# andvg3/LipVQ-VAE

Hardware: AMD Instinct MI355X
Metric: actions tokenized/sec (encode+quantize) at B=4096 T=128 K=1024, 1/2/4/8 GPU (higher is better)
Workload: dtype f32

## Files before the change

### lipvq-vae_amd/csrc/lipvq_screen.h

```cpp
#ifndef LIPVQ_SCREEN_H_
#define LIPVQ_SCREEN_H_
#include <hip/hip_fp16.h>

#include <type_traits>

#include "lipvq_common.h"

typedef _Float16 f16x8 __attribute__((ext_vector_type(8)));

#define LIPVQ_SCREEN_GAMMA 3.814697265625e-06f
#define SCREEN_WAVES 8

struct PrepLayout {
    int S, Dpad, Kpad, ntiles;
    size_t o_hdr, o_mu, o_tiles, tile_bytes, total;
    size_t o_tiles_hi, tile_bytes_hi;
};

#define LIPVQ_SCREEN_GAMMA_WIDE 1.52587890625e-05f
#define LQ_SCREEN_NARROW_MAX_S 13

__host__ __device__ static inline int lq_screen_S(int D) {
    const int s = (D + 15) / 16;
    return D <= 0 ? 0 : s <= 2 ? 2 : s <= 4 ? 4 : s <= 8 ? 8 : s <= 13 ? 13 : s <= 16 ? 16 : s <= 24 ? 24 : s <= 32 ? 32 : 0;
}
__host__ __device__ static inline float lq_screen_gamma(int D) {
    return lq_screen_S(D) > LQ_SCREEN_NARROW_MAX_S ? LIPVQ_SCREEN_GAMMA_WIDE : LIPVQ_SCREEN_GAMMA;
}

__host__ __device__ static inline PrepLayout prep_layout(int K, int D) {
    PrepLayout L;
    L.S = lq_screen_S(D) ? lq_screen_S(D) : (D + 15) / 16;
    L.Dpad = L.S * 16;
    L.Kpad = ((K + 31) / 32) * 32;
    L.ntiles = ((L.Kpad / 32 + 7) / 8) * 8;
    L.o_hdr = 0;
    L.o_mu = 64;
    L.o_tiles = L.o_mu + sizeof(float) * (size_t)L.Dpad;
    L.o_tiles = (L.o_tiles + 255) & ~(size_t)255;
    L.tile_bytes = (size_t)L.S * 2048 + 256;
    L.o_tiles_hi = (L.o_tiles + (size_t)L.ntiles * L.tile_bytes + 255) & ~(size_t)255;
    L.tile_bytes_hi = (size_t)L.S * 1024 + 256;
    L.total = L.o_tiles_hi + (size_t)L.ntiles * L.tile_bytes_hi;
    return L;
}


__device__ __forceinline__ int lq_scale_exp(float maxabs) {
    const int e = (int)((__float_as_uint(maxabs) >> 23) & 0xff) - 127;
    int k = 13 - e;
    k = k < -60 ? -60 : k;
    k = k > 60 ? 60 : k;
    return (maxabs > 0.0f && maxabs < INFINITY) ? k : 0;
}
__device__ __forceinline__ float lq_pow2f(int k) { return __uint_as_float((unsigned)(k + 127) << 23); }

constexpr int screen_default_tc(int S) { return (S <= 2) ? 8 : (S <= 4) ? 4 : (S <= 8) ? 2 : 1; }

template <int S, int TC_ = screen_default_tc(S), bool COARSE = false>
struct ScreenCfg {
    static constexpr int FRAG_BYTES = COARSE ? S * 1024 : S * 2048;
    static constexpr int TILE_BYTES = FRAG_BYTES + 256;
    static constexpr int TC = TC_;
    static constexpr int STAGE_BYTES = TC * TILE_BYTES;
    static constexpr int STAGE_VEC = STAGE_BYTES / 16;
};

template <int S>
struct StandaloneScreen {
    static constexpr int TC = (S <= 2) ? 4 : (S <= 4) ? 2 : 1;
    static constexpr int NB = (S <= 8) ? 4 : 3;
    static constexpr bool PACK = S <= 4;
};

template <bool PACK>
__device__ __forceinline__ void lq_track_one(float v, int id, unsigned keep_mask, float& m1, float& m2, int& k1) {
    if constexpr (PACK) {
        float key;
        asm("v_and_or_b32 %0, %1, %2, %3" : "=v"(key) : "v"(v), "s"(keep_mask), "v"(id));
        m2 = __builtin_amdgcn_fmed3f(key, m1, m2);
        asm("v_min_f32 %0, %1, %2" : "=v"(m1) : "v"(key), "v"(m1));
    } else {
        const bool lt = v < m1;
        k1 = lt ? id : k1;
        m2 = __builtin_amdgcn_fmed3f(v, m1, m2);
        m1 = lt ? v : m1;
    }
}

__device__ __forceinline__ float lq_coarse_zn(float a2lo, float n2, float fz, float fown, float rho) {
    const float A = lq_sqrt(a2lo), B = lq_sqrt(n2) * fz;
    const float t = lq_fma(rho, lq_fma(3.0f, A, B), A);
    return t * (fown / fz) * 1.0009765625f;
}
template <int LO, int HI, bool PACK = false, bool COARSE = false>
__device__ __forceinline__ void lq_track_part(const f32x16& acc, float e2, float en, const float (&frow)[16], const float (&znr)[16],
                                              int id, unsigned keep_mask, float (&m1)[16], float (&m2)[16], int (&k1)[16]) {
#pragma unroll
    for (int r = LO; r < HI; ++r) {
        const float v = COARSE ? acc[r] : lq_fma(e2, frow[r], acc[r]);
        lq_track_one<PACK>(v, id, keep_mask, m1[r], m2[r], k1[r]);
    }
}

template <int S, bool PACK, bool COARSE = false>
__device__ __forceinline__ void lq_track_after_mfma(int j, const f32x16& acc, float e2, float en, const float (&frow)[16],
                                                    const float (&znr)[16], int id, unsigned keep_mask, float (&m1)[16],
                                                    float (&m2)[16], int (&k1)[16]) {
    constexpr int NM = COARSE ? S : 3 * S;
    const int lo = (16 * j) / NM, hi = (16 * (j + 1)) / NM;
#pragma unroll
    for (int r = 0; r < 16; ++r)
        if (r >= lo && r < hi) {
            const float v = COARSE ? acc[r] : lq_fma(e2, frow[r], acc[r]);
            lq_track_one<PACK>(v, id, keep_mask, m1[r], m2[r], k1[r]);
        }
}

template <int N>
__device__ __forceinline__ void lq_wait_vmcnt() {
    static_assert(N >= 0 && N < 64, "vmcnt immediate");
    asm volatile("s_waitcnt vmcnt(%0)" ::"n"(N) : "memory");
}
template <int S, int TC_, int NB>
constexpr size_t lq_ring_bytes() { return (size_t)NB * ScreenCfg<S, TC_>::STAGE_BYTES + 1024; }

__host__ __device__ static inline int lq_pack_bits(int ntiles) { int b = 1; while ((1 << b) < ntiles) ++b; return b; }

struct LqNoDeferred { __device__ __forceinline__ void operator()() const {} };
template <int BASE, int NDEF, int NPF>
__device__ __forceinline__ void lq_wait_vmcnt_deferred(bool cd, bool cp) {
    static_assert(BASE + NDEF + NPF < 64, "vmcnt immediate");
    if (NDEF > 0 && NPF > 0 && cd && cp) lq_wait_vmcnt<BASE + NDEF + NPF>();
    else if (NDEF > 0 && cd) lq_wait_vmcnt<BASE + NDEF>();
    else if (NPF > 0 && cp) lq_wait_vmcnt<BASE + NPF>();
    else lq_wait_vmcnt<BASE>();
}
template <int S, int NT, int TC_ = screen_default_tc(S), int NB = 4, bool PACK = false, bool COARSE = false, int NDEF = 0,
          typename DEFERRED = LqNoDeferred, int NPF = 0>
__device__ __forceinline__ void lq_screen_core(const f16x8 (&ah)[S], const f16x8 (&al)[S],
                                               const unsigned char* __restrict__ tiles, int ntiles,
                                               unsigned char* stage0, int tid, const float (&frow)[16], const float (&znr)[16],
                                               float (&m1)[16], float (&m2)[16], int (&k1)[16],
                                               bool have_def = false, DEFERRED deferred = DEFERRED(), bool wave_def = true,
                                               bool have_pf = false) {
    using C = ScreenCfg<S, TC_, COARSE>;
    static_assert(NB >= 3 && NB <= 4, "ring of 3 or 4 stage buffers");
    constexpr int NW = NT / 64;
    constexpr int CHUNKS = (C::STAGE_BYTES + 1023) / 1024;
    constexpr int CPW = (CHUNKS + NW - 1) / NW;
    constexpr int PD = NB - 1;
    constexpr int NSTEP = C::TC * S;
    constexpr int MID = (C::TC >= 2) ? (C::TC / 2) * S : S / 2;
    constexpr int FR = 2;
    constexpr int FD = FR - 1;
    constexpr int PERIOD = ((C::TC & 1) || (NSTEP % FR)) ? 2 : 1;
    static_assert(C::STAGE_BYTES >= 1024 && C::STAGE_BYTES % 16 == 0, "stage copies are whole KiB pieces");
    static_assert(NSTEP - FD >= MID, "next-stage fragments are read after the hand-over");
    static_assert(CPW * PD < 64, "vmcnt immediate");
    const int lane = tid & 63, ln = lane & 31;
    const int wave = __builtin_amdgcn_readfirstlane(tid >> 6);
    const int nstage = ntiles / C::TC;
    unsigned char* dummy = stage0 + (size_t)NB * C::STAGE_BYTES;
    typedef __attribute__((address_space(3))) void* lds_ptr_t;
    typedef const __attribute__((address_space(1))) void* glb_ptr_t;
    auto stage_dma = [&](int st, int buf) {
        const bool real = st < nstage;
        const unsigned char* src = tiles + (real ? (size_t)st * C::STAGE_BYTES : (size_t)0);
        unsigned char* dst = stage0 + (size_t)buf * C::STAGE_BYTES;
#pragma unroll
        for (int j = 0; j < CPW; ++j) {
            int chunk = wave + j * NW;
            chunk = chunk < CHUNKS ? chunk : CHUNKS - 1;
            int off = chunk * 1024;
            off = off + 1024 <= C::STAGE_BYTES ? off : C::STAGE_BYTES - 1024;
            unsigned char* d = real ? dst + off : dummy;
            __builtin_amdgcn_global_load_lds((glb_ptr_t)(src + off + lane * 16), (lds_ptr_t)d, 16, 0, 0);
        }
    };
    auto frag = [&](const unsigned char* tb, int s, int hl) {
        return COARSE ? *reinterpret_cast<const f16x8*>(tb + ((size_t)s * 64 + lane) * 16)
                      : *reinterpret_cast<const f16x8*>(tb + (((size_t)s * 2 + hl) * 64 + lane) * 16);
    };
    lq_wg_barrier();
#pragma unroll
    for (int p = 0; p < PD; ++p) stage_dma(p, p);
    static_assert((PD - 1) * CPW + NDEF + NPF < 64, "vmcnt immediate");
    const bool count_def = NDEF > 0 && have_def && wave_def;
    const bool count_pf = NPF > 0 && have_pf;
    if ((NDEF > 0 && have_def) || count_pf) deferred();
    lq_wait_vmcnt_deferred<(PD - 1) * CPW, NDEF, NPF>(count_def, count_pf);
    lq_wg_barrier();

    f32x16 accA, accB;
#pragma unroll
    for (int r = 0; r < 16; ++r) accB[r] = INFINITY;
    float e2A = 0.0f, e2B = 0.0f;
    int codeA = 0, codeB = 0;
    const unsigned keep_mask = PACK ? ~((1u << lq_pack_bits(ntiles)) - 1u) : 0xffffffffu;
    f16x8 fh[FR], fl[FR];
    float e2q[2] = {0.0f, 0.0f};
    float enq[2] = {0.0f, 0.0f};
    float enA = 0.0f, enB = 0.0f;
#pragma unroll
    for (int g = 0; g < FD; ++g) {
        fh[g] = frag(stage0, g, 0);
        if constexpr (!COARSE) fl[g] = frag(stage0, g, 1);
    }
    e2q[0] = reinterpret_cast<const float*>(stage0 + C::FRAG_BYTES)[ln];
    if constexpr (COARSE) enq[0] = reinterpret_cast<const float*>(stage0 + C::FRAG_BYTES + 128)[ln];
    static_assert(FD <= S, "prologue reads stay in tile 0");
    int buf = 0;
    auto do_stage = [&](auto POS, int st) {
        constexpr int par = (decltype(POS)::value * C::TC) & 1;
        constexpr int so = (decltype(POS)::value * NSTEP) % FR;
        const unsigned char* sb = stage0 + (size_t)buf * C::STAGE_BYTES;
        int nbuf = buf + 1; nbuf = nbuf == NB ? 0 : nbuf;
        const unsigned char* nsb = stage0 + (size_t)nbuf * C::STAGE_BYTES;
#pragma unroll
        for (int g = 0; g < NSTEP; ++g) {
            const int c = g / S, s = g % S;
            if (g == MID) {
                if ((count_def || count_pf) && st == 0) lq_wait_vmcnt_deferred<(PD >= 2 ? (PD - 2) * CPW : 0), (PD >= 2 ? NDEF : 0), (PD >= 2 ? NPF : 0)>(count_def, count_pf);
                else lq_wait_vmcnt<(PD >= 2 ? (PD - 2) * CPW : 0)>();
                lq_wg_barrier();
                int b = buf + PD; b = b >= NB ? b - NB : b;
                stage_dma(st + PD, b);
            }
            f32x16& acc = (((c + par) & 1) == 0) ? accA : accB;
            const f32x16& prev = (((c + par) & 1) == 0) ? accB : accA;
            const float e2_prev = (((c + par) & 1) == 0) ? e2B : e2A;
            const float en_prev = (((c + par) & 1) == 0) ? enB : enA;
            const int code_prev = (((c + par) & 1) == 0) ? codeB : codeA;
            if (s == 0) {
                const float e2c = e2q[(c + par) & 1];
                const float enc = enq[(c + par) & 1];
#pragma unroll
                for (int r = 0; r < 16; ++r) acc[r] = COARSE ? lq_fma(-znr[r], enc, e2c * frow[r]) : 0.0f;
                int code = PACK ? (st * C::TC + c) : (st * C::TC + c) * 32 + ln;
                if constexpr (PACK) asm volatile("" : "+v"(code));
                if (((c + par) & 1) == 0) { e2A = e2c; enA = enc; codeA = code; } else { e2B = e2c; enB = enc; codeB = code; }
            }
            const f16x8 bh = fh[(g + so) % FR];
            f16x8 bl = bh;
            if constexpr (!COARSE) bl = fl[(g + so) % FR];
            auto read_ahead = [&]() {
                const int g1 = g + FD;
                const unsigned char* base = (g1 < NSTEP) ? sb : nsb;
                const int gg = (g1 < NSTEP) ? g1 : g1 - NSTEP;
                const unsigned char* tb = base + (size_t)(gg / S) * C::TILE_BYTES;
                fh[(g1 + so) % FR] = frag(tb, gg % S, 0);
                if constexpr (!COARSE) fl[(g1 + so) % FR] = frag(tb, gg % S, 1);
                if (gg % S == 0) {
                    e2q[(g1 / S + par) & 1] = reinterpret_cast<const float*>(tb + C::FRAG_BYTES)[ln];
                    if constexpr (COARSE) enq[(g1 / S + par) & 1] = reinterpret_cast<const float*>(tb + C::FRAG_BYTES + 128)[ln];
                }
            };
            __builtin_amdgcn_sched_barrier(0);
            acc = __builtin_amdgcn_mfma_f32_32x32x16_f16(ah[s], bh, acc, 0, 0, 0);
            __builtin_amdgcn_sched_barrier(0);
            read_ahead();
            __builtin_amdgcn_sched_barrier(0);
            lq_track_after_mfma<S, PACK, COARSE>(COARSE ? s : 3 * s + 0, prev, e2_prev, en_prev, frow, znr, code_prev, keep_mask, m1, m2, k1);
            __builtin_amdgcn_sched_barrier(0);
            if constexpr (!COARSE) {
                acc = __builtin_amdgcn_mfma_f32_32x32x16_f16(al[s], bh, acc, 0, 0, 0);
                lq_track_after_mfma<S, PACK>(3 * s + 1, prev, e2_prev, en_prev, frow, znr, code_prev, keep_mask, m1, m2, k1);
                __builtin_amdgcn_sched_barrier(0);
                acc = __builtin_amdgcn_mfma_f32_32x32x16_f16(ah[s], bl, acc, 0, 0, 0);
                lq_track_after_mfma<S, PACK>(3 * s + 2, prev, e2_prev, en_prev, frow, znr, code_prev, keep_mask, m1, m2, k1);
                __builtin_amdgcn_sched_barrier(0);
            }
        }
        buf = nbuf;
    };
    for (int st = 0; st < nstage; st += PERIOD) {
        do_stage(std::integral_constant<int, 0>{}, st);
        if constexpr (PERIOD == 2) do_stage(std::integral_constant<int, 1>{}, st + 1);
    }
    lq_track_part<0, 16, PACK, COARSE>(accB, e2B, enB, frow, znr, codeB, keep_mask, m1, m2, k1);
    lq_wait_vmcnt<0>();
    lq_wg_barrier();
}


__device__ __forceinline__ void lq_row_factors(float fown, int lane, float (&frow)[16]) {
    const int h = lane >> 5;
#pragma unroll
    for (int r = 0; r < 16; ++r) frow[r] = __shfl(fown, (r & 3) + 8 * (r >> 2) + 4 * h, 64);
}

#define LQ_DECIDE_STRIDE 36
#define LQ_DECIDE_BYTES (32 * LQ_DECIDE_STRIDE * 4)

struct LqDecision {
    float vv[16];
    float m2min, best, t0, p;
    bool screen_ok;
};

template <bool PACK = false, bool COARSE = false>
__device__ __forceinline__ bool lq_screen_decide(const float (&m1)[16], const float (&m2)[16], const int (&k1)[16],
                                                 unsigned char* wave_lds ,
                                                 const unsigned* hdr, float n2, float fown, float gamma, int K, int D,
                                                 int lane, int& my_k, LqDecision& dec, float pack_eps = 0.0f,
                                                 unsigned keep_mask = 0xffffffffu, float zn = 0.0f,
                                                 const unsigned char* tiles = nullptr, size_t tile_bytes = 0, int frag_bytes = 0) {
    constexpr int TS = LQ_DECIDE_STRIDE;
    const int ln = lane & 31, h = lane >> 5;
    float* tv = reinterpret_cast<float*>(wave_lds);
#pragma unroll
    for (int r = 0; r < 16; ++r) tv[((r & 3) + 8 * (r >> 2) + 4 * h) * TS + ln] = m1[r];
    __builtin_amdgcn_s_waitcnt(0xC07F);
    __builtin_amdgcn_wave_barrier();
    float best = INFINITY, second = INFINITY;
    int pos = 0;
    {
        const float4* pv = reinterpret_cast<const float4*>(tv + ln * TS + 16 * h);
#pragma unroll
        for (int q = 0; q < 4; ++q) {
            const float4 v4 = pv[q];
            const float vv[4] = {v4.x, v4.y, v4.z, v4.w};
#pragma unroll
            for (int e = 0; e < 4; ++e) {
                dec.vv[4 * q + e] = vv[e];
                const bool take = vv[e] < best;
                second = __builtin_amdgcn_fmed3f(vv[e], best, second);
                pos = take ? 4 * q + e : pos;
                best = take ? vv[e] : best;
            }
        }
    }
    __builtin_amdgcn_wave_barrier();
#pragma unroll
    for (int r = 0; r < 16; ++r) tv[((r & 3) + 8 * (r >> 2) + 4 * h) * TS + ln] = m2[r];
    __builtin_amdgcn_s_waitcnt(0xC07F);
    __builtin_amdgcn_wave_barrier();
    float m2min = INFINITY;
    {
        const float4* pv = reinterpret_cast<const float4*>(tv + ln * TS + 16 * h);
#pragma unroll
        for (int q = 0; q < 4; ++q) {
            const float4 v4 = pv[q];
            m2min = fminf(m2min, fminf(fminf(v4.x, v4.y), fminf(v4.z, v4.w)));
        }
    }
    second = fminf(second, m2min);
    __builtin_amdgcn_wave_barrier();
    int bk;
    if constexpr (PACK) {
        bk = (int)(__float_as_uint(best) & ~keep_mask) * 32 + 16 * h + pos;
    } else {
        int* tk = reinterpret_cast<int*>(wave_lds);
#pragma unroll
        for (int r = 0; r < 16; ++r) tk[((r & 3) + 8 * (r >> 2) + 4 * h) * TS + ln] = k1[r];
        __builtin_amdgcn_s_waitcnt(0xC07F);
        __builtin_amdgcn_wave_barrier();
        bk = tk[ln * TS + 16 * h + pos];
    }
    {
        const float ob = __shfl_xor(best, 32, 64);
        const float os = __shfl_xor(second, 32, 64);
        const int ok = __shfl_xor(bk, 32, 64);
        second = fminf(fminf(second, os), fmaxf(best, ob));
        const bool take = ob < best;
        bk = take ? ok : bk;
        best = take ? ob : best;
    }
    __builtin_amdgcn_wave_barrier();
    my_k = bk;
    const float E2max = __uint_as_float(hdr[0]);
    const float Emax = lq_sqrt(__uint_as_float(hdr[1]));
    const float twoemax = __uint_as_float(hdr[2]);
    const float cross = 2.0f * lq_sqrt(n2) * Emax;
    const int Dpad16 = ((D + 15) / 16) * 16 + ((D & 7) ? 88 : 0);
    const float u24 = 5.9604644775390625e-08f;
    const float eps_s = gamma * (E2max + cross) * fown;
    const float n2s = n2 * fown;
    float w2 = 0.0f;
    if constexpr (COARSE) {
        const int bkc = (bk >= 0 && bk < K) ? bk : 0;
        const float en = reinterpret_cast<const float*>(tiles + (size_t)(bkc >> 5) * tile_bytes + (size_t)frag_bytes + 128)[bkc & 31];
        w2 = 2.0f * zn * en;
        w2 = lq_fma(w2, 9.5367431640625e-07f, w2);
    }
    const float s1 = fmaxf(0.0f, best + w2 + n2s) + eps_s + (float)(Dpad16 + 2) * u24 * n2s;
    dec.t0 = w2 + 2.0f * eps_s + 2.125f * (float)(Dpad16 / 8 + 12) * u24 * s1;
    dec.p = 2.125f * pack_eps;
    dec.best = best;
    dec.m2min = m2min;
    dec.screen_ok = (twoemax < INFINITY) && (bk >= 0) && (bk < K);
    const float thr = dec.t0 + dec.p * (lq_abs(best) + lq_abs(second));
    return dec.screen_ok && (second - best > thr);
}

#define LQ_CAND_MAX 6

#define LQ_STREAM2_MIN_S 9
struct LqWorkspace {
    unsigned char* base;
    int64_t N;
    int D;

    static constexpr int kHeaderBytes = 64, kLive = 8, kSlot2 = kLive + 2;
    __host__ __device__ static inline LqWorkspace from_lists(int* row_list, int64_t N) {
        return LqWorkspace{reinterpret_cast<unsigned char*>(row_list) - kHeaderBytes, N, 0};
    }
    __host__ __device__ static inline LqWorkspace from_live(int* live) {
        return LqWorkspace{reinterpret_cast<unsigned char*>(live - kLive), 0, 0};
    }
    __host__ __device__ static inline size_t list_ints(int64_t N) { return ((size_t)N + 15) & ~(size_t)15; }
    __host__ __device__ static inline size_t short_cap(int64_t N) { return (size_t)N + 64; }
    __host__ __device__ static inline size_t w2q_floats(int D) {
        return (D + 15) / 16 >= LQ_STREAM2_MIN_S ? (size_t)((D + 31) / 32) * 16 * 256 : 0;
    }
    __host__ __device__ static inline size_t lists_end(int64_t N) {
        return kHeaderBytes + sizeof(int) * (3 * list_ints(N) + 16 * short_cap(N));
    }
    __host__ __device__ static inline size_t nearest_bytes(int64_t N) { return lists_end(N); }
    __host__ __device__ static inline size_t tokenize_bytes(int64_t N, int D) {
        return lists_end(N) + sizeof(float) * w2q_floats(D) + 256 + sizeof(float) * (size_t)N * (size_t)D;
    }

    __host__ __device__ inline int* header() const { return reinterpret_cast<int*>(base); }
    __host__ __device__ inline int* published() const { return header(); }
    __host__ __device__ inline const int* listed() const { return header() + 1; }
    __host__ __device__ inline int* live() const { return header() + kLive; }
    __host__ __device__ inline int* slot2_count() const { return header() + kSlot2; }
    __host__ __device__ inline int* row_list() const { return reinterpret_cast<int*>(base + kHeaderBytes); }
    __host__ __device__ inline int* best_list() const { return row_list() + list_ints(N); }
    __host__ __device__ inline int* short_lists() const { return row_list() + 2 * list_ints(N); }
    __host__ __device__ inline size_t short_cap() const { return short_cap(N); }
    __host__ __device__ inline int* slot2_list() const { return row_list() + (2 * list_ints(N) + 16 * short_cap(N)); }
    __host__ __device__ inline float* w2q() const { return reinterpret_cast<float*>(base + lists_end(N)); }
    __host__ __device__ inline float* ze_scratch() const {
        return reinterpret_cast<float*>(base + ((lists_end(N) + sizeof(float) * w2q_floats(D) + 255) & ~(size_t)255));
    }
    __host__ __device__ inline long long* stamps() const { return reinterpret_cast<long long*>(row_list() + (N / 2 & ~1)); }
};

#if defined(__HIPCC__)
__device__ __forceinline__ void lq_ws_begin(int* __restrict__ live) {
    if (blockIdx.x == 0 && threadIdx.x == 0) *LqWorkspace::from_live(live).slot2_count() = 0;
}
__device__ __forceinline__ void lq_ws_publish(int* __restrict__ live) {
    asm volatile("s_waitcnt vmcnt(0)" ::: "memory");
    __syncthreads();
    if (threadIdx.x == 0) {
        const unsigned long long old = atomicAdd(reinterpret_cast<unsigned long long*>(live), 1ull << 32);
        if ((unsigned)(old >> 32) == gridDim.x - 1u) {
            const int listed = (int)(unsigned)old;
            int* published = LqWorkspace::from_live(live).published();
            published[0] = listed;
            published[1] = listed;
            *reinterpret_cast<unsigned long long*>(live) = 0ull;
        }
    }
}
__device__ __forceinline__ int lq_ws_reserve(int* __restrict__ live, int n) {
    return (int)(unsigned)atomicAdd(reinterpret_cast<unsigned long long*>(live), (unsigned long long)(unsigned)n);
}
#endif

template <bool PACK>
__device__ __forceinline__ void lq_emit_candidates(const LqDecision& dec, bool lists_ok, int K, int lane, unsigned keep_mask,
                                                   const unsigned char* wave_lds, int& head, unsigned& mask_out,
                                                   int (&codes)[LQ_CAND_MAX]) {
    const int ln = lane & 31, h = lane >> 5;
    const float ab = lq_abs(dec.best);
    const float vmax0 = (dec.best + dec.t0 + dec.p * ab) / (1.0f - dec.p);
    const float vmax = vmax0 + lq_abs(vmax0) * 9.5367431640625e-07f + 1.1754944e-38f;
    int n = 0;
    unsigned mask = 0u;
    bool nothing = !lists_ok || !dec.screen_ok || !(vmax == vmax);
    const bool second_in = !(dec.m2min - dec.best > dec.t0 + dec.p * (ab + lq_abs(dec.m2min)));
#pragma unroll
    for (int q = 0; q < LQ_CAND_MAX; ++q) codes[q] = 0;
#pragma unroll
    for (int e = 0; e < 16; ++e) {
        const float v = dec.vv[e];
        if (!(v > vmax)) mask |= 1u << e;
        if (!(v - dec.best > dec.t0 + dec.p * (ab + lq_abs(v)))) {
            int code;
            if constexpr (PACK) code = (int)(__float_as_uint(v) & ~keep_mask) * 32 + 16 * h + e;
            else code = reinterpret_cast<const int*>(wave_lds)[ln * LQ_DECIDE_STRIDE + 16 * h + e];
            nothing = nothing || code < 0 || code >= K;
#pragma unroll
            for (int q = 0; q < LQ_CAND_MAX; ++q)
                if (q == n) codes[q] = code;
            ++n;
        }
    }
    head = nothing ? -1 : ((second_in || n > LQ_CAND_MAX) ? -2 : n);
    mask_out = mask;
}

__device__ __forceinline__ void lq_emit_store(bool need, int slot , int head, unsigned mask,
                                              const int (&codes)[LQ_CAND_MAX], int my_k, int64_t row, int* __restrict__ amb_list,
                                              int64_t N, int lane) {
    const int h = lane >> 5;
    const LqWorkspace ws = LqWorkspace::from_lists(amb_list, N);
    if (h == 0 && need) {
        ws.row_list()[slot] = (int)row;
        ws.best_list()[slot] = my_k;
    }
    if (!need || (size_t)slot >= ws.short_cap()) return;
    int* out = ws.short_lists() + (size_t)slot * 16 + 8 * h;
    static_assert(LQ_CAND_MAX == 6, "a part is {n, mask, six codes}");
    typedef int lq_i4 __attribute__((ext_vector_type(4)));
    lq_i4* out4 = reinterpret_cast<lq_i4*>(out);
    out4[0] = lq_i4{head, (int)mask, codes[0], codes[1]};
    out4[1] = lq_i4{codes[2], codes[3], codes[4], codes[5]};
}

#define LQ_SLOT_HEAD(cl, h) ((cl)[8 * (h)])
#define LQ_SLOT_SHORT(n0, n1) ((n0) >= 0 && (n1) >= 0 && (n0) + (n1) >= 1 && (n0) <= LQ_CAND_MAX && (n1) <= LQ_CAND_MAX)
#define LQ_SLOT_CODE(cl, n0, j) ((j) < (n0) ? (cl)[2 + (j)] : (cl)[10 + ((j) - (n0))])
#define LQ_SLOT_FIRST(cl, n0) ((cl)[(n0) > 0 ? 2 : 10])
#define LQ_SLOT_LANES(cl) (((unsigned)(cl)[1] & 0xffffu) | (((unsigned)(cl)[9] & 0xffffu) << 16))

template <bool PACK>
__device__ __forceinline__ void lq_screen_emit(const LqDecision& dec, bool certified, bool lists_ok, int my_k, int64_t row,
                                               bool row_valid, int* __restrict__ amb_count, int* __restrict__ amb_list, int64_t N,
                                               int K, int lane, unsigned keep_mask, const unsigned char* wave_lds) {
    const bool need = row_valid && !certified;
    if (__builtin_amdgcn_ballot_w64(need) == 0ull) return;
    const int ln = lane & 31, h = lane >> 5;
    const unsigned long long lm = __builtin_amdgcn_ballot_w64(h == 0 && need);
    const int leader = __builtin_ctzll(lm);
    int base = 0;
    if (lane == leader) base = lq_ws_reserve(amb_count, __builtin_popcountll(lm));
    int head;
    unsigned mask;
    int codes[LQ_CAND_MAX];
    lq_emit_candidates<PACK>(dec, lists_ok, K, lane, keep_mask, wave_lds, head, mask, codes);
    base = __shfl(base, leader, 64);
    int slot = base + __builtin_popcountll(lm & ((1ull << lane) - 1ull));
    slot = __shfl(slot, ln, 64);
    lq_emit_store(need, slot, head, mask, codes, my_k, row, amb_list, N, lane);
}

#define LQ_LISTS_ALL_K 2048
template <int DCH, int DIST, typename ZLOAD>
__device__ __forceinline__ int lq_lists_row(ZLOAD zload, const float* __restrict__ cb, int K, const int* cl, int lane, bool all_here) {
    constexpr int D = DCH * 8;
    const int g = lane >> 3, j = lane & 7;
    int n0 = -1, n1 = -1;
    if (cl) { n0 = LQ_SLOT_HEAD(cl, 0); n1 = LQ_SLOT_HEAD(cl, 1); }
    const bool shortlist = LQ_SLOT_SHORT(n0, n1);
    const bool lanescan = !shortlist && n0 != -1 && n1 != -1 && (n0 == -2 || n1 == -2 || n0 > LQ_CAND_MAX || n1 > LQ_CAND_MAX);
    const unsigned lmask = lanescan ? LQ_SLOT_LANES(cl) : 0u;
    bool scan_here = lanescan && lmask != 0u && __builtin_popcount(lmask) * ((K + 31) / 32) <= 128;
    unsigned lm_eff = lmask;
    if (!shortlist && !scan_here) {
        if (!all_here) return -1;
        scan_here = true;
        lm_eff = (lanescan && lmask != 0u) ? lmask : 0xffffffffu;
    }
    const bool scanning = !shortlist;
    const int P = scanning ? __builtin_popcount(lm_eff) : 0;
    const int nc = scanning ? P * ((K + 31) / 32) : n0 + n1;
    float zv[DCH];
#pragma unroll
    for (int i = 0; i < DCH; ++i) zv[i] = zload(8 * i + j);
    float best_v = INFINITY;
    int best_k = 0x7fffffff;
    for (int c0 = 0; c0 < nc; c0 += 8) {
        const int ci = c0 + g;
        bool live = ci < nc;
        int code;
        if (scanning) {
            const int t = ci / P, w = ci - t * P;
            unsigned m = lm_eff;
            for (int q = 0; q < w; ++q) m &= m - 1;
            code = 32 * t + __builtin_ctz(m | 0x80000000u);
            live = live && code < K;
        } else {
            code = live ? LQ_SLOT_CODE(cl, n0, ci) : LQ_SLOT_FIRST(cl, n0);
        }
        code = (code >= 0 && code < K) ? code : 0;
        const float* c = cb + (size_t)code * D;
        float s;
        if constexpr (DIST == LIPVQ_DIST_NORM) {
            float a = 0.0f;
#pragma unroll
            for (int i = 0; i < DCH; ++i) { const float d = zv[i] - c[8 * i + j]; a = lq_fma(d, d, a); }
            s = __shfl(a, 8 * g, 64);
#pragma unroll
            for (int l = 1; l < 8; ++l) s = s + __shfl(a, 8 * g + l, 64);
            s = lq_sqrt(s);
        } else {
            float acc[4] = {0.f, 0.f, 0.f, 0.f};
#pragma unroll
            for (int i = 0; i < DCH; ++i) {
                const int q = (i < (DCH / 4) * 4) ? (i & 3) : 0;
                const float d = zv[i] - c[8 * i + j];
                acc[q] = acc[q] + d * d;
            }
            const float vl = ((acc[0] + acc[1]) + acc[2]) + acc[3];
            s = __shfl(vl, 8 * g, 64);
#pragma unroll
            for (int l = 1; l < 8; ++l) s = s + __shfl(vl, 8 * g + l, 64);
        }
        const float v = (live && s == s) ? s : INFINITY;
        const int kk = live ? code : 0x7fffffff;
        LQ_TAKE_MIN(best_v, best_k, v, kk);
    }
    LQ_WAVE_MIN(best_v, best_k, 8);
    if (best_k < 0 || best_k >= K) {
        const int fb = scanning ? __builtin_ctz(lm_eff) : LQ_SLOT_FIRST(cl, n0);
        best_k = (fb >= 0 && fb < K) ? fb : 0;
    }
    return best_k;
}

template <bool PACK, int DCH, int DIST, int NKEEP = 0>
__device__ __forceinline__ bool lq_screen_decide_inplace(const LqDecision& dec, bool certified, bool lists_ok, int& my_k, int64_t row0,
                                                         bool row_valid, int* __restrict__ amb_count, const float* __restrict__ z,
                                                         const float* __restrict__ cb, int K, int lane, unsigned keep_mask,
                                                         unsigned char* wave_lds ,
                                                         const f32x16* zkeep = nullptr) {
    const bool need = row_valid && !certified;
    if (__builtin_amdgcn_ballot_w64(need) == 0ull) return certified;
    const int ln = lane & 31, h = lane >> 5;
    unsigned long long lm = __builtin_amdgcn_ballot_w64(h == 0 && need);
    if (lane == __builtin_ctzll(lm)) (void)lq_ws_reserve(amb_count, __builtin_popcountll(lm));
    int head;
    unsigned mask;
    int codes[LQ_CAND_MAX];
    lq_emit_candidates<PACK>(dec, lists_ok, K, lane, keep_mask, wave_lds, head, mask, codes);
    __builtin_amdgcn_wave_barrier();
    int* parts = reinterpret_cast<int*>(wave_lds);
    static_assert(LQ_CAND_MAX == 6 && 32 * 16 * 4 <= LQ_DECIDE_BYTES, "a part is {n, mask, six codes}");
    if (need) {
        typedef int lq_i4 __attribute__((ext_vector_type(4)));
        lq_i4* out4 = reinterpret_cast<lq_i4*>(parts + ln * 16 + 8 * h);
        out4[0] = lq_i4{head, (int)mask, codes[0], codes[1]};
        out4[1] = lq_i4{codes[2], codes[3], codes[4], codes[5]};
    }
    __builtin_amdgcn_s_waitcnt(0xC07F);
    __builtin_amdgcn_wave_barrier();
    constexpr int D = DCH * 8;
    while (lm) {
        const int r = __builtin_ctzll(lm);
        lm &= lm - 1ull;
        int bk;
        if constexpr (NKEEP > 0) {
            static_assert(NKEEP * 32 == D, "the kept tiles are the row");
            float* zrow = reinterpret_cast<float*>(wave_lds + LQ_DECIDE_BYTES);
            if (ln == r) {
#pragma unroll
                for (int t = 0; t < NKEEP; ++t)
#pragma unroll
                    for (int q = 0; q < 16; ++q) zrow[32 * t + 2 * q + h] = zkeep[t][q];
            }
            __builtin_amdgcn_s_waitcnt(0xC07F);
            __builtin_amdgcn_wave_barrier();
            bk = lq_lists_row<DCH, DIST>([&](int f) { return zrow[f]; }, cb, K, parts + r * 16, lane, true);
            __builtin_amdgcn_wave_barrier();
        } else {
            const float* zr = z + (size_t)(row0 + r) * D;
            bk = lq_lists_row<DCH, DIST>([&](int f) { return __hip_atomic_load(zr + f, __ATOMIC_RELAXED, __HIP_MEMORY_SCOPE_AGENT); },
                                         cb, K, parts + r * 16, lane, true);
        }
        if (ln == r) { my_k = bk; certified = true; }
    }
    __builtin_amdgcn_wave_barrier();
    return certified;
}

struct LqGatherTrip { float4 val[8]; };
__device__ __forceinline__ void lq_gather_load(LqGatherTrip& g, const float* __restrict__ cb, int my_k, bool row_ok, int64_t row0,
                                               int64_t N, int D, int lane, int trip) {
    const int nvec = D / 4;
    const int v = 16 * trip + (lane & 15);
    const int vc = v < nvec ? v : nvec - 1;
#pragma unroll
    for (int p = 0; p < 8; ++p) {
        const int src_lane = 4 * p + (lane >> 4);
        const int kk = __shfl(my_k, src_lane, 64);
        const bool ok = (__shfl((int)row_ok, src_lane, 64) != 0) && (row0 + src_lane < N);
        g.val[p] = reinterpret_cast<const float4*>(cb + (size_t)(ok ? kk : 0) * D)[vc];
    }
}
__device__ __forceinline__ void lq_gather_store(const LqGatherTrip& g, float* __restrict__ zq, bool row_ok, int64_t row0, int64_t N,
                                                int D, int lane, int trip) {
    const int nvec = D / 4;
    const int v = 16 * trip + (lane & 15);
#pragma unroll
    for (int p = 0; p < 8; ++p) {
        const int src_lane = 4 * p + (lane >> 4);
        const bool ok = (__shfl((int)row_ok, src_lane, 64) != 0) && (row0 + src_lane < N) && (v < nvec);
        if (ok) reinterpret_cast<float4*>(zq + (size_t)(row0 + src_lane) * D)[v] = g.val[p];
    }
}
template <int NP>
__device__ __forceinline__ void lq_gather_dma(unsigned char* wave_stage, const float* __restrict__ cb, int my_k, bool row_ok,
                                              int64_t row0, int64_t N, int D, int lane, int trip, int p0) {
    typedef __attribute__((address_space(3))) void* lds_ptr_t;
    typedef const __attribute__((address_space(1))) void* glb_ptr_t;
    const int nvec = D / 4;
    const int v = 16 * trip + (lane & 15);
    const int vc = v < nvec ? v : nvec - 1;
#pragma unroll
    for (int p = 0; p < NP; ++p) {
        const int src_lane = 4 * (p0 + p) + (lane >> 4);
        const int kk = __shfl(my_k, src_lane, 64);
        const bool ok = (__shfl((int)row_ok, src_lane, 64) != 0) && (row0 + src_lane < N);
        const float4* src = reinterpret_cast<const float4*>(cb + (size_t)(ok ? kk : 0) * D) + vc;
        __builtin_amdgcn_global_load_lds((glb_ptr_t)src, (lds_ptr_t)(wave_stage + p * 1024), 16, 0, 0);
    }
}
template <int NP>
__device__ __forceinline__ void lq_gather_flush(const unsigned char* wave_stage, float* __restrict__ zq, bool row_ok, int64_t row0,
                                                int64_t N, int D, int lane, int trip, int p0) {
    const int nvec = D / 4;
    const int v = 16 * trip + (lane & 15);
#pragma unroll
    for (int p = 0; p < NP; ++p) {
        const int src_lane = 4 * (p0 + p) + (lane >> 4);
        const bool ok = (__shfl((int)row_ok, src_lane, 64) != 0) && (row0 + src_lane < N) && (v < nvec);
        const float4 val = *reinterpret_cast<const float4*>(wave_stage + p * 1024 + lane * 16);
        typedef float lq_f4v __attribute__((ext_vector_type(4)));
        if (ok) __builtin_nontemporal_store((lq_f4v){val.x, val.y, val.z, val.w}, reinterpret_cast<lq_f4v*>(zq + (size_t)(row0 + src_lane) * D) + v);
    }
}
__device__ __forceinline__ void lq_screen_gather(const float* __restrict__ cb, float* __restrict__ zq, int my_k,
                                                 bool certified, int64_t row0, int64_t N, int D, int lane) {
    if (D & 3) {
        for (int p = 0; p < 8; ++p) {
            const int src_lane = 4 * p + (lane >> 4);
            const int kk = __shfl(my_k, src_lane, 64);
            const bool ok = (__shfl((int)certified, src_lane, 64) != 0) && (row0 + src_lane < N);
            if (ok)
                for (int d = lane & 15; d < D; d += 16) zq[(size_t)(row0 + src_lane) * D + d] = cb[(size_t)kk * D + d];
        }
        return;
    }
    for (int trip = 0; 64 * trip < D; ++trip) {
        LqGatherTrip g;
        lq_gather_load(g, cb, my_k, certified, row0, N, D, lane, trip);
        lq_gather_store(g, zq, certified, row0, N, D, lane, trip);
    }
}

static inline int lq_screen_coarse_default(int S, int K) { return (K >= 4096 || (S >= 8 && K >= 1024)) ? 1 : 0; }
int lq_screen_coarse(int S, int K);

struct LqOut {
    int64_t* idx;
    float* zq;
    int64_t* usage;
};
int lipvq_launch_rows(const float* z, int z_by_slot, const float* cb, const LqOut& out, const LqWorkspace& ws, int K, hipStream_t st,
                      int dist = LIPVQ_DIST_NORM);
int lipvq_launch_rows_encode(const float* x, const float* const* raw6, int A, const float* cb, const LqOut& out, const LqWorkspace& ws,
                             int K, hipStream_t st);
#endif
```

Measured before the change: 1.401 billion.

## Unroll screen ring statically and hoist DMA address math out of stage loop

For small packed screens (S<=4), the loop over the stage ring is unrolled one full pass at a time, so buffer indices become compile-time constants. DMA chunk offsets are precomputed once. Real-versus-dummy destinations are chosen with branchless masks on a running past counter, and LDS fragment and norm reads use 32-bit LDS addresses. Min tracking for this case is split across two MFMA slots instead of three, with the fma, pack and track steps batched into separate passes. The aim is to cut scalar and vector address overhead and shorten the tracking chain between MFMAs, at the cost of a larger code size and more intricate pointer arithmetic.

```diff
diff --git a/lipvq-vae_amd/csrc/lipvq_screen.h b/lipvq-vae_amd/csrc/lipvq_screen.h
--- a/lipvq-vae_amd/csrc/lipvq_screen.h
+++ b/lipvq-vae_amd/csrc/lipvq_screen.h
@@ -73,13 +73,14 @@
     static constexpr bool PACK = S <= 4;
 };
 
+__device__ __forceinline__ float lq_pack_key(float v, int id, unsigned keep_mask) {
+    return __uint_as_float((__float_as_uint(v) & keep_mask) | (unsigned)id);
+}
 template <bool PACK>
 __device__ __forceinline__ void lq_track_one(float v, int id, unsigned keep_mask, float& m1, float& m2, int& k1) {
     if constexpr (PACK) {
-        float key;
-        asm("v_and_or_b32 %0, %1, %2, %3" : "=v"(key) : "v"(v), "s"(keep_mask), "v"(id));
-        m2 = __builtin_amdgcn_fmed3f(key, m1, m2);
-        asm("v_min_f32 %0, %1, %2" : "=v"(m1) : "v"(key), "v"(m1));
+        m2 = __builtin_amdgcn_fmed3f(v, m1, m2);
+        asm("v_min_f32 %0, %1, %2" : "=v"(m1) : "v"(v), "v"(m1));
     } else {
         const bool lt = v < m1;
         k1 = lt ? id : k1;
@@ -99,22 +100,34 @@
 #pragma unroll
     for (int r = LO; r < HI; ++r) {
         const float v = COARSE ? acc[r] : lq_fma(e2, frow[r], acc[r]);
-        lq_track_one<PACK>(v, id, keep_mask, m1[r], m2[r], k1[r]);
-    }
-}
-
-template <int S, bool PACK, bool COARSE = false>
-__device__ __forceinline__ void lq_track_after_mfma(int j, const f32x16& acc, float e2, float en, const float (&frow)[16],
+        lq_track_one<PACK>(PACK ? lq_pack_key(v, id, keep_mask) : v, id, keep_mask, m1[r], m2[r], k1[r]);
+    }
+}
+
+template <int NG, bool PACK, bool COARSE = false>
+__device__ __forceinline__ void lq_track_after_mfma(int q, const f32x16& acc, float e2, float en, const float (&frow)[16],
                                                     const float (&znr)[16], int id, unsigned keep_mask, float (&m1)[16],
                                                     float (&m2)[16], int (&k1)[16]) {
-    constexpr int NM = COARSE ? S : 3 * S;
-    const int lo = (16 * j) / NM, hi = (16 * (j + 1)) / NM;
-#pragma unroll
-    for (int r = 0; r < 16; ++r)
-        if (r >= lo && r < hi) {
-            const float v = COARSE ? acc[r] : lq_fma(e2, frow[r], acc[r]);
-            lq_track_one<PACK>(v, id, keep_mask, m1[r], m2[r], k1[r]);
-        }
+    const int lo = (16 * q) / NG, hi = (16 * (q + 1)) / NG;
+    if constexpr (PACK && !COARSE) {
+        float key[16];
+#pragma unroll
+        for (int r = 0; r < 16; ++r)
+            if (r >= lo && r < hi) key[r] = lq_fma(e2, frow[r], acc[r]);
+#pragma unroll
+        for (int r = 0; r < 16; ++r)
+            if (r >= lo && r < hi) key[r] = lq_pack_key(key[r], id, keep_mask);
+#pragma unroll
+        for (int r = 0; r < 16; ++r)
+            if (r >= lo && r < hi) lq_track_one<PACK>(key[r], id, keep_mask, m1[r], m2[r], k1[r]);
+    } else {
+#pragma unroll
+        for (int r = 0; r < 16; ++r)
+            if (r >= lo && r < hi) {
+                const float v = COARSE ? acc[r] : lq_fma(e2, frow[r], acc[r]);
+                lq_track_one<PACK>(PACK ? lq_pack_key(v, id, keep_mask) : v, id, keep_mask, m1[r], m2[r], k1[r]);
+            }
+    }
 }
 
 template <int N>
@@ -154,37 +167,53 @@
     constexpr int MID = (C::TC >= 2) ? (C::TC / 2) * S : S / 2;
     constexpr int FR = 2;
     constexpr int FD = FR - 1;
+    constexpr bool BOOK2 = PACK && !COARSE && S <= 4;
+    constexpr bool RING_STATIC = BOOK2 && (8 / C::TC) % NB == 0;
     constexpr int PERIOD = ((C::TC & 1) || (NSTEP % FR)) ? 2 : 1;
     static_assert(C::STAGE_BYTES >= 1024 && C::STAGE_BYTES % 16 == 0, "stage copies are whole KiB pieces");
     static_assert(NSTEP - FD >= MID, "next-stage fragments are read after the hand-over");
     static_assert(CPW * PD < 64, "vmcnt immediate");
     const int lane = tid & 63, ln = lane & 31;
     const int wave = __builtin_amdgcn_readfirstlane(tid >> 6);
-    const int nstage = ntiles / C::TC;
+    const int nstage = __builtin_amdgcn_readfirstlane(ntiles / C::TC);
     unsigned char* dummy = stage0 + (size_t)NB * C::STAGE_BYTES;
     typedef __attribute__((address_space(3))) void* lds_ptr_t;
     typedef const __attribute__((address_space(1))) void* glb_ptr_t;
-    auto stage_dma = [&](int st, int buf) {
-        const bool real = st < nstage;
-        const unsigned char* src = tiles + (real ? (size_t)st * C::STAGE_BYTES : (size_t)0);
-        unsigned char* dst = stage0 + (size_t)buf * C::STAGE_BYTES;
+    int poff[CPW];
+#pragma unroll
+    for (int j = 0; j < CPW; ++j) {
+        int chunk = wave + j * NW;
+        chunk = chunk < CHUNKS ? chunk : CHUNKS - 1;
+        const int off = chunk * 1024;
+        poff[j] = off + 1024 <= C::STAGE_BYTES ? off : C::STAGE_BYTES - 1024;
+    }
+    const unsigned lane16 = (unsigned)lane * 16u;
+    auto stage_dma = [&](int past, size_t src_off, int rp) {
+        const int real = __builtin_amdgcn_readfirstlane(past >> 31);
+        const size_t real64 = ((size_t)(unsigned)real << 32) | (unsigned)real;
+        const unsigned char* src = tiles + (src_off & real64);
+        unsigned char* dbase = dummy - ((NB - rp) * C::STAGE_BYTES & real);
 #pragma unroll
         for (int j = 0; j < CPW; ++j) {
-            int chunk = wave + j * NW;
-            chunk = chunk < CHUNKS ? chunk : CHUNKS - 1;
-            int off = chunk * 1024;
-            off = off + 1024 <= C::STAGE_BYTES ? off : C::STAGE_BYTES - 1024;
-            unsigned char* d = real ? dst + off : dummy;
-            __builtin_amdgcn_global_load_lds((glb_ptr_t)(src + off + lane * 16), (lds_ptr_t)d, 16, 0, 0);
-        }
+            unsigned char* d = dbase + (poff[j] & real);
+            __builtin_amdgcn_global_load_lds((glb_ptr_t)(src + poff[j] + lane16), (lds_ptr_t)d, 16, 0, 0);
+        }
+    };
+    typedef const __attribute__((address_space(3))) float* lds_cfloat_t;
+    typedef const __attribute__((address_space(3))) f16x8* lds_cfrag_t;
+    unsigned norm_lane = (unsigned)(uintptr_t)(lds_ptr_t)(stage0 + C::FRAG_BYTES + ln * 4);
+    unsigned frag_lane = (unsigned)(uintptr_t)(lds_ptr_t)(stage0 + lane * 16);
+    if constexpr (RING_STATIC) asm volatile("" : "+v"(norm_lane), "+v"(frag_lane));
+    auto norm_at = [&](const unsigned char* tb, int extra) {
+        return *(lds_cfloat_t)(uintptr_t)(norm_lane + (unsigned)(tb - stage0) + (unsigned)extra);
     };
     auto frag = [&](const unsigned char* tb, int s, int hl) {
-        return COARSE ? *reinterpret_cast<const f16x8*>(tb + ((size_t)s * 64 + lane) * 16)
-                      : *reinterpret_cast<const f16x8*>(tb + (((size_t)s * 2 + hl) * 64 + lane) * 16);
+        const int piece = COARSE ? s : s * 2 + hl;
+        return *(lds_cfrag_t)(uintptr_t)(frag_lane + (unsigned)(tb - stage0) + (unsigned)piece * 1024u);
     };
     lq_wg_barrier();
 #pragma unroll
-    for (int p = 0; p < PD; ++p) stage_dma(p, p);
+    for (int p = 0; p < PD; ++p) stage_dma(p - nstage, (size_t)p * C::STAGE_BYTES, p);
     static_assert((PD - 1) * CPW + NDEF + NPF < 64, "vmcnt immediate");
     const bool count_def = NDEF > 0 && have_def && wave_def;
     const bool count_pf = NPF > 0 && have_pf;
@@ -207,25 +236,30 @@
         fh[g] = frag(stage0, g, 0);
         if constexpr (!COARSE) fl[g] = frag(stage0, g, 1);
     }
-    e2q[0] = reinterpret_cast<const float*>(stage0 + C::FRAG_BYTES)[ln];
-    if constexpr (COARSE) enq[0] = reinterpret_cast<const float*>(stage0 + C::FRAG_BYTES + 128)[ln];
+    e2q[0] = norm_at(stage0, 0);
+    if constexpr (COARSE) enq[0] = norm_at(stage0, 128);
     static_assert(FD <= S, "prologue reads stay in tile 0");
     int buf = 0;
-    auto do_stage = [&](auto POS, int st) {
+    int past = PD - nstage;
+    size_t src_off = (size_t)PD * C::STAGE_BYTES;
+    auto do_stage = [&](auto POS, auto RP, auto FIRST, int st) {
         constexpr int par = (decltype(POS)::value * C::TC) & 1;
         constexpr int so = (decltype(POS)::value * NSTEP) % FR;
-        const unsigned char* sb = stage0 + (size_t)buf * C::STAGE_BYTES;
-        int nbuf = buf + 1; nbuf = nbuf == NB ? 0 : nbuf;
-        const unsigned char* nsb = stage0 + (size_t)nbuf * C::STAGE_BYTES;
+        const int rp = RP;
+        const unsigned char* sb = stage0 + (size_t)rp * C::STAGE_BYTES;
+        int nrp = rp + 1; nrp = nrp == NB ? 0 : nrp;
+        const unsigned char* nsb = stage0 + (size_t)nrp * C::STAGE_BYTES;
 #pragma unroll
         for (int g = 0; g < NSTEP; ++g) {
             const int c = g / S, s = g % S;
             if (g == MID) {
-                if ((count_def || count_pf) && st == 0) lq_wait_vmcnt_deferred<(PD >= 2 ? (PD - 2) * CPW : 0), (PD >= 2 ? NDEF : 0), (PD >= 2 ? NPF : 0)>(count_def, count_pf);
+                if ((count_def || count_pf) && FIRST) lq_wait_vmcnt_deferred<(PD >= 2 ? (PD - 2) * CPW : 0), (PD >= 2 ? NDEF : 0), (PD >= 2 ? NPF : 0)>(count_def, count_pf);
                 else lq_wait_vmcnt<(PD >= 2 ? (PD - 2) * CPW : 0)>();
                 lq_wg_barrier();
-                int b = buf + PD; b = b >= NB ? b - NB : b;
-                stage_dma(st + PD, b);
+                int b = rp + PD; b = b >= NB ? b - NB : b;
+                stage_dma(past, src_off, b);
+                past += 1;
+                src_off += C::STAGE_BYTES;
             }
             f32x16& acc = (((c + par) & 1) == 0) ? accA : accB;
             const f32x16& prev = (((c + par) & 1) == 0) ? accB : accA;
@@ -252,8 +286,8 @@
                 fh[(g1 + so) % FR] = frag(tb, gg % S, 0);
                 if constexpr (!COARSE) fl[(g1 + so) % FR] = frag(tb, gg % S, 1);
                 if (gg % S == 0) {
-                    e2q[(g1 / S + par) & 1] = reinterpret_cast<const float*>(tb + C::FRAG_BYTES)[ln];
-                    if constexpr (COARSE) enq[(g1 / S + par) & 1] = reinterpret_cast<const float*>(tb + C::FRAG_BYTES + 128)[ln];
+                    e2q[(g1 / S + par) & 1] = norm_at(tb, 0);
+                    if constexpr (COARSE) enq[(g1 / S + par) & 1] = norm_at(tb, 128);
                 }
             };
             __builtin_amdgcn_sched_barrier(0);
@@ -261,22 +295,38 @@
             __builtin_amdgcn_sched_barrier(0);
             read_ahead();
             __builtin_amdgcn_sched_barrier(0);
-            lq_track_after_mfma<S, PACK, COARSE>(COARSE ? s : 3 * s + 0, prev, e2_prev, en_prev, frow, znr, code_prev, keep_mask, m1, m2, k1);
+            if constexpr (!BOOK2) lq_track_after_mfma<COARSE ? S : 3 * S, PACK, COARSE>(COARSE ? s : 3 * s + 0, prev, e2_prev, en_prev, frow, znr, code_prev, keep_mask, m1, m2, k1);
             __builtin_amdgcn_sched_barrier(0);
             if constexpr (!COARSE) {
+                constexpr int NG = BOOK2 ? 2 * S : 3 * S;
                 acc = __builtin_amdgcn_mfma_f32_32x32x16_f16(al[s], bh, acc, 0, 0, 0);
-                lq_track_after_mfma<S, PACK>(3 * s + 1, prev, e2_prev, en_prev, frow, znr, code_prev, keep_mask, m1, m2, k1);
+                lq_track_after_mfma<NG, PACK>(BOOK2 ? 2 * s + 0 : 3 * s + 1, prev, e2_prev, en_prev, frow, znr, code_prev, keep_mask, m1, m2, k1);
                 __builtin_amdgcn_sched_barrier(0);
                 acc = __builtin_amdgcn_mfma_f32_32x32x16_f16(ah[s], bl, acc, 0, 0, 0);
-                lq_track_after_mfma<S, PACK>(3 * s + 2, prev, e2_prev, en_prev, frow, znr, code_prev, keep_mask, m1, m2, k1);
+                lq_track_after_mfma<NG, PACK>(BOOK2 ? 2 * s + 1 : 3 * s + 2, prev, e2_prev, en_prev, frow, znr, code_prev, keep_mask, m1, m2, k1);
                 __builtin_amdgcn_sched_barrier(0);
             }
         }
-        buf = nbuf;
     };
-    for (int st = 0; st < nstage; st += PERIOD) {
-        do_stage(std::integral_constant<int, 0>{}, st);
-        if constexpr (PERIOD == 2) do_stage(std::integral_constant<int, 1>{}, st + 1);
+    if constexpr (RING_STATIC) {
+        static_assert(NB == 4 && NB % PERIOD == 0, "one trip = one pass of the ring");
+        auto ring_pass = [&](auto FIRST, int st) {
+            do_stage(std::integral_constant<int, 0>{}, std::integral_constant<int, 0>{}, FIRST, st);
+            do_stage(std::integral_constant<int, 1 % PERIOD>{}, std::integral_constant<int, 1>{}, std::false_type{}, st + 1);
+            do_stage(std::integral_constant<int, 2 % PERIOD>{}, std::integral_constant<int, 2>{}, std::false_type{}, st + 2);
+            do_stage(std::integral_constant<int, 3 % PERIOD>{}, std::integral_constant<int, 3>{}, std::false_type{}, st + 3);
+        };
+        ring_pass(std::true_type{}, 0);
+        for (int st = NB; st < nstage; st += NB) ring_pass(std::false_type{}, st);
+    } else {
+        for (int st = 0; st < nstage; st += PERIOD) {
+            do_stage(std::integral_constant<int, 0>{}, buf, st == 0, st);
+            buf = buf + 1 == NB ? 0 : buf + 1;
+            if constexpr (PERIOD == 2) {
+                do_stage(std::integral_constant<int, 1>{}, buf, false, st + 1);
+                buf = buf + 1 == NB ? 0 : buf + 1;
+            }
+        }
     }
     lq_track_part<0, 16, PACK, COARSE>(accB, e2B, enB, frow, znr, codeB, keep_mask, m1, m2, k1);
     lq_wait_vmcnt<0>();
```

Measured after the change: 1.420 billion (median of 6 runs). +1.4%, better.
